# 3dhumangan/3DHumanGAN

Hardware: NVIDIA H100
Metric: images_per_sec_G_fwd_512x512 (higher is better)
Workload: dtype f32 (bf16x3 split on wgmma, fp32 accumulate)

## Files before the change

### 3dhumangan_b200/csrc/synth.cu

```cuda
#include "common.cuh"
#include "wgmma.cuh"

namespace hg {

constexpr int kC = 256;
constexpr int kSynThreads = 384;
constexpr int kSynStages = 2;
constexpr int kASlots = 2;
constexpr int kXSlots = 5;
constexpr int kXs = 3;
constexpr int kSs = 2;
constexpr uint32_t kAChunk = 128 * 128;
constexpr uint32_t kBStage = 256 * 128;
constexpr uint32_t kXSlice = 32 * 128 * 4;

struct SpadeArgs {
  const float* x;
  long x_bstride;
  const float* mod;
  const float* scsh;
  const float* p_lr;
  long p_stride;
  const float* p_bias;
  const uint8_t* wgb;
  const float* bgb;
  const uint8_t* wimg;
  const float* bias;
  const float* skip;
  long skip_bstride;
  float* out;
  double* stats;
  const float* rgb_w;
  const float* rgb_b;
  const float* rgb_in;
  float* rgb_out;
  int B, HW, Hg, Wg, Rh, Rw;
  int nkc;
  int xC;
  const float* x2;
  float slope;
  int cout;
  int out_pm;
  int act;
  const float* ascale;
  const float* rk_v;
  int rk_n;
  const float* mod2;
};

struct SynSmem {
  uint8_t* a_hi;
  uint8_t* a_lo;
  uint8_t* b_st;
  float* x_st;
  int xs_n, ss_n;
  float* tab_g1;
  float* tab_g0;
  float* tab_bias;
  float* tab_rgbw;
  float* tab_bgb;
  float* tab_as;
  float* st_sum;
  float* st_sq;
  uint64_t* bars;
};

template <bool kPixel>
__device__ __forceinline__ SynSmem carve(uint8_t* raw) {
  constexpr int kA = kPixel ? 3 : kASlots, kX = kPixel ? 3 : kXSlots;
  uint8_t* s = reinterpret_cast<uint8_t*>((reinterpret_cast<uintptr_t>(raw) + 1023) & ~uintptr_t(1023));
  SynSmem m;
  m.a_hi = s;
  m.a_lo = s + kA * kAChunk;
  m.b_st = s + 2 * kA * kAChunk;
  m.x_st = reinterpret_cast<float*>(m.b_st + kSynStages * kBStage);
  m.xs_n = kPixel ? 2 : kXs;
  m.ss_n = kPixel ? 1 : kSs;
  float* f = m.x_st + kX * (kXSlice / 4);
  m.tab_g1 = f; f += kC;
  m.tab_g0 = f; f += kC;
  m.tab_bias = f; f += kC;
  m.tab_rgbw = f; f += 3 * kC;
  m.tab_bgb = f; f += 512;
  m.tab_as = f; f += kC;
  m.st_sum = f; f += kC;
  m.st_sq = f; f += kC;
  m.bars = reinterpret_cast<uint64_t*>(f);
  return m;
}
constexpr uint32_t kSynSmemBytes = 2 * kASlots * kAChunk + kSynStages * kBStage + kXSlots * kXSlice +
                                   (kC * 9 + 512) * 4 + 24 * 8 + 1024;
constexpr uint32_t kPixSmemBytes = 2 * 3 * kAChunk + kSynStages * kBStage + 3 * kXSlice + (kC * 9 + 512) * 4 + 24 * 8 + 1024;
static_assert(kSynSmemBytes <= 232448 && kPixSmemBytes <= 232448, "shared memory budget");

enum { B_FULL = 0 , B_EMPTY = 2 , X_FULL = 4 , X_EMPTY = 12  };

__device__ __forceinline__ void rows_barrier() { named_barrier(1, 256); }

__device__ __forceinline__ float lrelu02(float v) { return v > 0.f ? v : 0.2f * v; }

__device__ __forceinline__ float reduce_2pi(float t) {
  const float y = t * 0.15915494309189535f;
  const float k = (y + 12582912.f) - 12582912.f;
  float r = fmaf(-k, 6.2831854820251465f, t);
  return fmaf(-k, -1.7484555314695172e-07f, r);
}
__device__ __forceinline__ float sin_red(float t) { return __sinf(reduce_2pi(t)); }
__device__ __forceinline__ float cos_red(float t) { return __cosf(reduce_2pi(t)); }
__device__ __forceinline__ float2 reduce_2pi2(float2 t) {
  const float2 y = fmul2(t, make_float2(0.15915494309189535f, 0.15915494309189535f));
  const float2 k = fadd2(fadd2(y, make_float2(12582912.f, 12582912.f)), make_float2(-12582912.f, -12582912.f));
  const float2 r = ffma2(k, make_float2(-6.2831854820251465f, -6.2831854820251465f), t);
  return ffma2(k, make_float2(1.7484555314695172e-07f, 1.7484555314695172e-07f), r);
}
__device__ __forceinline__ float2 sin_red2(float2 t) { const float2 r = reduce_2pi2(t); return make_float2(__sinf(r.x), __sinf(r.y)); }
__device__ __forceinline__ float2 cos_red2(float2 t) { const float2 r = reduce_2pi2(t); return make_float2(__cosf(r.x), __cosf(r.y)); }

struct TileMap {
  int T, first, stride, count;
  __device__ __forceinline__ void get(int it, int& b, int& ti) const {
    const int tile = first + it * stride;
    b = tile / T;
    ti = tile - b * T;
  }
};

__device__ __forceinline__ void init_common(const SpadeArgs& a, const SynSmem& m) {
  for (int i = threadIdx.x; i < kC; i += blockDim.x) {
    m.tab_bias[i] = a.bias[i];
    m.st_sum[i] = 0.f;
    m.st_sq[i] = 0.f;
  }
  if (a.rgb_w)
    for (int i = threadIdx.x; i < 3 * kC; i += blockDim.x) m.tab_rgbw[i] = a.rgb_w[i];
  if (threadIdx.x == 0) {
    for (int i = 0; i < kSynStages; ++i) {
      mbar_init(m.bars + B_FULL + i, 1);
      mbar_init(m.bars + B_EMPTY + i, 2);
    }
    for (int i = 0; i < m.xs_n + m.ss_n; ++i) {
      mbar_init(m.bars + X_FULL + i, 1);
      mbar_init(m.bars + X_EMPTY + i, 8);
    }
    fence_mbar_init();
  }
  __syncthreads();
}

template <int kPasses>
__device__ __forceinline__ void weight_producer_loop(const SynSmem& m, const uint8_t* img, int nstages, int num_my_tiles) {
  uint32_t st = 0, ph = 0;
  for (int t = 0; t < num_my_tiles; ++t)
    for (int s = 0; s < nstages; ++s) {
      if (kPasses == 1 && (s & 1)) continue;
      mbar_wait_backoff(m.bars + B_EMPTY + st, ph ^ 1);
      mbar_arrive_expect_tx(m.bars + B_FULL + st, kBStage);
      bulk_g2s(m.b_st + st * kBStage, img + static_cast<size_t>(s) * kBStage, kBStage, m.bars + B_FULL + st);
      if (++st == kSynStages) { st = 0; ph ^= 1; }
    }
}

struct Pipe {
  uint32_t st = 0, ph = 0, prev = ~0u;
};
template <int N, int kPasses>
__device__ __forceinline__ void pipe_chunk(const SynSmem& m, Pipe& p, float (&d)[N / 2], uint32_t a_hi, uint32_t a_lo, bool accumulate,
                                           int t) {
#pragma unroll
  for (int part = 0; part < (kPasses == 3 ? 2 : 1); ++part) {
    mbar_wait(m.bars + B_FULL + p.st, p.ph);
    acc_fence(d);
    wgmma_fence();
    const uint32_t bt = smem_u32(m.b_st + p.st * kBStage);
    if (part == 0) {
      wg_k64<N>(d, a_hi, bt, accumulate);
      if (kPasses == 3) wg_k64<N>(d, a_lo, bt, true);
    } else {
      wg_k64<N>(d, a_hi, bt, true);
    }
    wgmma_commit();
    wgmma_wait<1>();
    acc_fence(d);
    if (p.prev != ~0u && t == 0) mbar_arrive(m.bars + B_EMPTY + p.prev);
    p.prev = p.st;
    if (++p.st == kSynStages) { p.st = 0; p.ph ^= 1; }
  }
}
template <int N>
__device__ __forceinline__ void pipe_drain(const SynSmem& m, Pipe& p, float (&d)[N / 2], int t) {
  wgmma_wait<0>();
  acc_fence(d);
  if (p.prev != ~0u && t == 0) mbar_arrive(m.bars + B_EMPTY + p.prev);
  p.prev = ~0u;
}

__device__ __forceinline__ void ring_emit(const SynSmem& m, uint32_t& g, int base, int slots, const float* src) {
  const uint32_t slot = base + g % slots;
  mbar_wait_backoff(m.bars + X_EMPTY + slot, ((g / slots) & 1) ^ 1);
  mbar_arrive_expect_tx(m.bars + X_FULL + slot, kXSlice);
  bulk_g2s(m.x_st + slot * (kXSlice / 4), src, kXSlice, m.bars + X_FULL + slot);
  ++g;
}
__device__ __forceinline__ void x_producer_loop(const SpadeArgs& a, const SynSmem& m, const TileMap& tm) {
  uint32_t g = 0;
  for (int it = 0; it < tm.count; ++it) {
    int b, ti;
    tm.get(it, b, ti);
    const int per_src = a.xC / 32;
    const float* base = a.x + static_cast<long>(b) * a.x_bstride + static_cast<long>(ti) * a.xC * 128;
    const float* base2 = a.x2 ? a.x2 + (static_cast<long>(b) * tm.T + ti) * a.xC * 128 : nullptr;
    for (int j = 0; j < 2 * a.nkc; ++j)
      ring_emit(m, g, 0, m.xs_n, (j < per_src ? base : base2 - per_src * 32 * 128) + j * 32 * 128);
  }
}
__device__ __forceinline__ void skip_producer_loop(const SpadeArgs& a, const SynSmem& m, const TileMap& tm) {
  if (!a.skip) return;
  uint32_t g = 0;
  for (int it = 0; it < tm.count; ++it) {
    int b, ti;
    tm.get(it, b, ti);
    const float* base = a.skip + static_cast<long>(b) * a.skip_bstride + static_cast<long>(ti) * a.cout * 128;
    for (int j = 0; j < a.cout / 32; ++j) ring_emit(m, g, m.xs_n, m.ss_n, base + j * 32 * 128);
  }
}

__device__ __forceinline__ uint32_t ring_take(const SynSmem& m, uint32_t g, int base, int slots) {
  const uint32_t slot = base + g % slots;
  mbar_wait_sleep(m.bars + X_FULL + slot, (g / slots) & 1);
  return slot;
}
__device__ __forceinline__ void ring_release(const SynSmem& m, uint32_t slot) {
  __syncwarp();
  if ((threadIdx.x & 31) == 0) mbar_arrive(m.bars + X_EMPTY + slot);
}

__device__ __forceinline__ void take_x_pair(const SynSmem& m, uint32_t& xg, int h, int row, float (&dst)[32]) {
#pragma unroll
  for (int hh = 0; hh < 2; ++hh, ++xg) {
    const uint32_t xslot = ring_take(m, xg, 0, m.xs_n);
    if (hh == h) {
      const uint32_t xs = smem_u32(m.x_st + xslot * (kXSlice / 4)) + row * 4;
#pragma unroll
      for (int j = 0; j < 32; ++j) dst[j] = lds_f32(xs + j * 512);
    }
    ring_release(m, xslot);
  }
}

__device__ __forceinline__ void column_sums(float* st, int c0, const float (&v)[4][2]) {
  const int lane = threadIdx.x & 31, r = lane >> 2;
  const bool b2 = r & 4, b1 = r & 2, b0 = r & 1;
  float w[4], u[2];
#pragma unroll
  for (int i = 0; i < 4; ++i) {
    const float lo = v[i >> 1][i & 1], hi = v[(i + 4) >> 1][i & 1];
    w[i] = (b2 ? hi : lo) + __shfl_xor_sync(0xffffffffu, b2 ? lo : hi, 16);
  }
#pragma unroll
  for (int i = 0; i < 2; ++i)
    u[i] = (b1 ? w[i + 2] : w[i]) + __shfl_xor_sync(0xffffffffu, b1 ? w[i] : w[i + 2], 8);
  const float x = (b0 ? u[1] : u[0]) + __shfl_xor_sync(0xffffffffu, b0 ? u[0] : u[1], 4);
  atomicAdd(st + c0 + 8 * (r >> 1) + 2 * (lane & 3) + (r & 1), x);
}

template <bool kSkip>
__device__ __forceinline__ void epilogue_fwd(const SpadeArgs& a, const SynSmem& m, const float (&d)[128], int b, int ti, int T,
                                             int g, int t, uint32_t& sg) {
  const int HW = a.HW, cout = a.cout;
  const bool kRgb = a.rgb_w != nullptr, kStats = a.stats != nullptr;
  int row[2];
  bool valid[2];
#pragma unroll
  for (int i = 0; i < 2; ++i) {
    row[i] = g * 64 + frag_row(t, i);
    valid[i] = ti * 128 + row[i] < HW;
  }
  float* const otile = a.out + (static_cast<long>(b) * T + ti) * cout * 128;
  float r[2][3] = {{0.f, 0.f, 0.f}, {0.f, 0.f, 0.f}};
#pragma unroll
  for (int cg = 0; cg < 8; ++cg) {
    if (cg * 32 >= cout) break;
    float sk[2][4][2];
    if (kSkip) {
      const uint32_t slot = ring_take(m, sg, m.xs_n, m.ss_n);
      const float* xs = m.x_st + slot * (kXSlice / 4);
#pragma unroll
      for (int i = 0; i < 2; ++i)
#pragma unroll
        for (int jj = 0; jj < 4; ++jj)
#pragma unroll
          for (int e = 0; e < 2; ++e) sk[i][jj][e] = xs[(frag_col(t, jj, e)) * 128 + row[i]];
      ring_release(m, slot);
      ++sg;
    }
    float s1[4][2], s2[4][2];
#pragma unroll
    for (int jj = 0; jj < 4; ++jj)
#pragma unroll
      for (int e = 0; e < 2; ++e) {
        const int j = cg * 4 + jj, c = frag_col(t, j, e);
        const float bc = m.tab_bias[c];
        s1[jj][e] = 0.f;
        s2[jj][e] = 0.f;
#pragma unroll
        for (int i = 0; i < 2; ++i) {
          float v = d[4 * j + 2 * i + e] + bc;
          if (kSkip) v += sk[i][jj][e];
          if (valid[i]) otile[c * 128 + row[i]] = v;
          else v = 0.f;
          if (kRgb) {
#pragma unroll
            for (int k = 0; k < 3; ++k) r[i][k] = fmaf(v, m.tab_rgbw[k * kC + c], r[i][k]);
          }
          s1[jj][e] += v;
          s2[jj][e] = fmaf(v, v, s2[jj][e]);
        }
      }
    if (kStats) {
      column_sums(m.st_sum, cg * 32, s1);
      column_sums(m.st_sq, cg * 32, s2);
    }
  }
  if (kRgb) {
#pragma unroll
    for (int i = 0; i < 2; ++i) {
#pragma unroll
      for (int k = 0; k < 3; ++k) {
        r[i][k] += __shfl_xor_sync(0xffffffffu, r[i][k], 1);
        r[i][k] += __shfl_xor_sync(0xffffffffu, r[i][k], 2);
      }
      if ((t & 3) == 0 && valid[i]) {
        const int pix = ti * 128 + row[i];
#pragma unroll
        for (int k = 0; k < 3; ++k) {
          const long idx = (static_cast<long>(b) * 3 + k) * HW + pix;
          float o = r[i][k] + a.rgb_b[k];
          if (a.rgb_in) o += a.rgb_in[idx];
          a.rgb_out[idx] = o;
        }
      }
    }
  }
}

__device__ __forceinline__ void epilogue_fwd_any(const SpadeArgs& a, const SynSmem& m, const float (&d)[128], int b, int ti, int T,
                                                 int g, int t, uint32_t& sg) {
  if (a.skip) epilogue_fwd<true>(a, m, d, b, ti, T, g, t, sg);
  else epilogue_fwd<false>(a, m, d, b, ti, T, g, t, sg);
}

__device__ __forceinline__ void flush_fwd_stats(const SpadeArgs& a, const SynSmem& m) {
  rows_barrier();
  if (a.stats)
    for (int c = threadIdx.x; c < kC; c += 256) {
      atomicAdd(a.stats + c, static_cast<double>(m.st_sum[c]));
      atomicAdd(a.stats + kC + c, static_cast<double>(m.st_sq[c]));
    }
}

template <bool kSine, bool kRk, bool kPm>
__device__ __forceinline__ void epilogue_bwd(const SpadeArgs& a, const SynSmem& m, const float (&d)[128], int b, int ti, int T, int g,
                                             int t, uint32_t& sg) {
  const int HW = a.HW, cout = a.cout, rk_n = a.rk_n;
  const float mslope = a.slope;
  int row[2];
  bool valid[2];
  float rv[2][3] = {{0.f, 0.f, 0.f}, {0.f, 0.f, 0.f}};
#pragma unroll
  for (int i = 0; i < 2; ++i) {
    row[i] = g * 64 + frag_row(t, i);
    valid[i] = ti * 128 + row[i] < HW;
    if (kRk && valid[i]) {
      const float* rp = a.rk_v + static_cast<long>(b) * rk_n * HW + ti * 128 + row[i];
      rv[i][0] = rp[0];
      if (rk_n > 1) rv[i][1] = rp[HW];
      if (rk_n > 2) rv[i][2] = rp[2 * static_cast<long>(HW)];
    }
  }
  float* const otile = a.out + (static_cast<long>(b) * T + ti) * cout * 128;
#pragma unroll
  for (int cg = 0; cg < 8; ++cg) {
    if (cg * 32 >= cout) break;
    float xv[2][4][2];
    {
      const uint32_t slot = ring_take(m, sg, m.xs_n, m.ss_n);
      const float* xs = m.x_st + slot * (kXSlice / 4);
#pragma unroll
      for (int i = 0; i < 2; ++i)
#pragma unroll
        for (int jj = 0; jj < 4; ++jj)
#pragma unroll
          for (int e = 0; e < 2; ++e)
            xv[i][jj][e] = valid[i] ? xs[frag_col(t, jj, e) * 128 + row[i]] : 0.f;
      ring_release(m, slot);
      ++sg;
    }
    float s1[4][2], s2[4][2];
#pragma unroll
    for (int jj = 0; jj < 4; ++jj)
#pragma unroll
      for (int e = 0; e < 2; ++e) {
        const int j = cg * 4 + jj, c = frag_col(t, j, e);
        const float t1 = m.tab_g1[c], t0 = m.tab_g0[c];
        s1[jj][e] = 0.f;
        s2[jj][e] = 0.f;
#pragma unroll
        for (int i = 0; i < 2; ++i) {
          const float x = xv[i][jj][e];
          const float pre = fmaf(x, t1, t0);
          float acc = d[4 * j + 2 * i + e];
          if (kRk)
            acc = fmaf(rv[i][2], m.tab_rgbw[2 * kC + c], fmaf(rv[i][1], m.tab_rgbw[kC + c], fmaf(rv[i][0], m.tab_rgbw[c], acc)));
          const float mask = kSine ? cos_red(pre) : (pre > 0.f ? 1.f : mslope);
          const float dd = acc * mask;
          if (valid[i]) {
            if (kPm) a.out[(static_cast<long>(b) * HW + ti * 128 + row[i]) * cout + c] = dd;
            else otile[c * 128 + row[i]] = dd;
          }
          s1[jj][e] += dd;
          s2[jj][e] = fmaf(dd, x, s2[jj][e]);
        }
      }
    column_sums(m.st_sum, cg * 32, s1);
    column_sums(m.st_sq, cg * 32, s2);
  }
}

__device__ __forceinline__ void epilogue_bwd_any(const SpadeArgs& a, const SynSmem& m, const float (&d)[128], int b, int ti, int T,
                                                 int g, int t, uint32_t& sg) {
  if (a.act == 1) {
    if (a.rk_v) epilogue_bwd<true, true, false>(a, m, d, b, ti, T, g, t, sg);
    else epilogue_bwd<true, false, false>(a, m, d, b, ti, T, g, t, sg);
  } else {
    if (a.out_pm) epilogue_bwd<false, false, true>(a, m, d, b, ti, T, g, t, sg);
    else epilogue_bwd<false, false, false>(a, m, d, b, ti, T, g, t, sg);
  }
}

__device__ __forceinline__ void flush_bwd_sums(const SpadeArgs& a, const SynSmem& m, int b) {
  for (int c = threadIdx.x; c < a.cout; c += 256) {
    atomicAdd(a.stats + (static_cast<long>(b) * 2 + 0) * a.cout + c, static_cast<double>(m.st_sum[c]));
    atomicAdd(a.stats + (static_cast<long>(b) * 2 + 1) * a.cout + c, static_cast<double>(m.st_sq[c]));
    m.st_sum[c] = 0.f;
    m.st_sq[c] = 0.f;
  }
}

template <int kPasses, bool kBwd>
__global__ void __launch_bounds__(kSynThreads, 1) spade_const_kernel(SpadeArgs a) {
  extern __shared__ uint8_t smem_raw[];
  const SynSmem m = carve<false>(smem_raw);
  const int warp = threadIdx.x >> 5, lane = threadIdx.x & 31;
  init_common(a, m);
  TileMap tm;
  tm.T = (a.HW + 127) / 128;
  tm.first = blockIdx.x;
  tm.stride = gridDim.x;
  tm.count = (a.B * tm.T - static_cast<int>(blockIdx.x) + static_cast<int>(gridDim.x) - 1) / static_cast<int>(gridDim.x);

  if (warp < 8) {
    regs_inc<kMmaRegs>();
    const int g = warp >> 2, t = threadIdx.x & 127;
    const int q = 2 * g + (warp & 1), h = (warp >> 1) & 1;
    const int row = q * 32 + lane;
    int cur_b = -1;
    uint32_t acnt = 0;
    uint32_t xg = 0, sg = 0;
    Pipe p;
    float d[128];
    for (int it = 0; it < tm.count; ++it) {
      int b, ti;
      tm.get(it, b, ti);
      if (b != cur_b) {
        rows_barrier();
        if (kBwd && cur_b >= 0) flush_bwd_sums(a, m, cur_b);
        for (int i = threadIdx.x; i < kC; i += 256) {
          if (kBwd) {
            if (a.ascale) {
              const long ld = a.x2 ? 2 * kC : kC;
              m.tab_as[i] = a.ascale[static_cast<long>(b) * ld + i];
              if (a.x2) m.tab_bgb[i] = a.ascale[static_cast<long>(b) * ld + kC + i];
            }
            if (i < a.cout) {
              m.tab_g1[i] = a.mod ? a.mod[(static_cast<long>(b) * 2 + 0) * a.cout + i] : 1.f;
              m.tab_g0[i] = a.mod ? a.mod[(static_cast<long>(b) * 2 + 1) * a.cout + i] : 0.f;
            }
          } else {
            m.tab_g1[i] = a.mod ? a.mod[(static_cast<long>(b) * 2 + 0) * kC + i] : 1.f;
            m.tab_g0[i] = a.mod ? a.mod[(static_cast<long>(b) * 2 + 1) * kC + i] : 0.f;
            if (a.mod2) {
              m.tab_bgb[i] = a.mod2[(static_cast<long>(b) * 2 + 0) * kC + i];
              m.tab_bgb[kC + i] = a.mod2[(static_cast<long>(b) * 2 + 1) * kC + i];
            }
          }
        }
        rows_barrier();
        cur_b = b;
      }
      const bool valid = ti * 128 + row < a.HW;
      uint32_t tg1a = smem_u32(kBwd ? m.tab_as : m.tab_g1), tg0a = smem_u32(m.tab_g0);
      uint32_t tg1b = smem_u32(m.tab_bgb), tg0b = smem_u32(m.tab_bgb + kC);
      opaque(tg1a);
      opaque(tg0a);
      opaque(tg1b);
      opaque(tg0b);
      const float slope = a.slope;
      const bool sine = a.act == 1, scaled = kBwd && a.ascale != nullptr;
      const bool two_tables = kBwd ? (scaled && a.x2 != nullptr) : a.mod2 != nullptr;
#pragma unroll 1
      for (int kc = 0; kc < a.nkc; ++kc, ++acnt) {
        const int c0 = (kc * 64 + h * 32) & (kC - 1);
        const bool second = two_tables && kc * 64 >= kC;
        const uint32_t tg1 = second ? tg1b : tg1a, tg0 = second ? tg0b : tg0a;
        float cur[32];
        take_x_pair(m, xg, h, row, cur);
        const uint32_t slot = acnt & 1;
#pragma unroll
        for (int gi = 0; gi < 4; ++gi) {
          float y[8], t1[8], t0[8];
          if (!kBwd || scaled) lds8(tg1 + (c0 + gi * 8) * 4, t1);
          if (!kBwd) lds8(tg0 + (c0 + gi * 8) * 4, t0);
          if (kBwd) {
#pragma unroll
            for (int j = 0; j < 8; ++j) y[j] = scaled ? cur[gi * 8 + j] * t1[j] : cur[gi * 8 + j];
          } else if (sine) {
#pragma unroll
            for (int j = 0; j < 8; j += 2) {
              const float2 sv = sin_red2(ffma2(make_float2(cur[gi * 8 + j], cur[gi * 8 + j + 1]), make_float2(t1[j], t1[j + 1]),
                                               make_float2(t0[j], t0[j + 1])));
              y[j] = sv.x;
              y[j + 1] = sv.y;
            }
          } else {
            affine_lrelu8(cur + gi * 8, t1, t0, slope, y);
          }
          if (!valid) {
#pragma unroll
            for (int j = 0; j < 8; ++j) y[j] = 0.f;
          }
          store_a8<kPasses == 3>(m.a_hi + slot * kAChunk, m.a_lo + slot * kAChunk, row, h * 32 + gi * 8, y);
        }
        fence_proxy_async_smem();
        named_barrier(2 + g, 128);
        pipe_chunk<256, kPasses>(m, p, d, smem_u32(m.a_hi + slot * kAChunk) + g * 64 * 128,
                                 smem_u32(m.a_lo + slot * kAChunk) + g * 64 * 128, kc > 0, t);
      }
      pipe_drain<256>(m, p, d, t);
      if (kBwd) epilogue_bwd_any(a, m, d, b, ti, tm.T, g, t, sg);
      else epilogue_fwd_any(a, m, d, b, ti, tm.T, g, t, sg);
    }
    if (kBwd) {
      rows_barrier();
      if (cur_b >= 0) flush_bwd_sums(a, m, cur_b);
    } else {
      flush_fwd_stats(a, m);
    }
  } else {
    regs_dec<kProducerRegs>();
    if (lane == 0) {
      if (warp == 8) weight_producer_loop<kPasses>(m, a.wimg, 2 * a.nkc, tm.count);
      else if (warp == 9) x_producer_loop(a, m, tm);
      else if (warp == 10) skip_producer_loop(a, m, tm);
    }
  }
}

__device__ __forceinline__ void bilin(int dst, int in_size, float scale, int& i0, int& i1, float& l0, float& l1) {
  float src = scale * (static_cast<float>(dst) + 0.5f) - 0.5f;
  src = src < 0.f ? 0.f : src;
  i0 = static_cast<int>(src);
  i1 = i0 + (i0 < in_size - 1 ? 1 : 0);
  l1 = src - static_cast<float>(i0);
  l0 = 1.f - l1;
}

template <int kPasses>
__device__ __forceinline__ void pixel_weight_producer_loop(const SpadeArgs& a, const SynSmem& m, int num_my_tiles) {
  uint32_t st = 0, ph = 0;
  auto emit = [&](const uint8_t* src, uint32_t bytes) {
    mbar_wait_backoff(m.bars + B_EMPTY + st, ph ^ 1);
    mbar_arrive_expect_tx(m.bars + B_FULL + st, bytes);
    bulk_g2s(m.b_st + st * kBStage, src, bytes, m.bars + B_FULL + st);
    if (++st == kSynStages) { st = 0; ph ^= 1; }
  };
  for (int t = 0; t < num_my_tiles; ++t)
    for (int kc = 0; kc < 4; ++kc) {
      for (int k = 0; k < 2; ++k)
        for (int part = 0; part < (kPasses == 3 ? 2 : 1); ++part)
          emit(a.wgb + static_cast<size_t>(((kc >> 1) * 2 + k) * 2 + part) * kBStage + (kc & 1) * (kBStage / 2), kBStage / 2);
      for (int part = 0; part < (kPasses == 3 ? 2 : 1); ++part) emit(a.wimg + static_cast<size_t>(kc * 2 + part) * kBStage, kBStage);
    }
}

template <int kPasses>
__global__ void __launch_bounds__(kSynThreads, 1) spade_pixel_kernel(SpadeArgs a) {
  extern __shared__ uint8_t smem_raw[];
  const SynSmem m = carve<true>(smem_raw);
  const int warp = threadIdx.x >> 5, lane = threadIdx.x & 31;
  for (int i = threadIdx.x; i < kC; i += blockDim.x) {
    m.tab_g1[i] = a.scsh[i];
    m.tab_g0[i] = a.scsh[kC + i];
  }
  for (int i = threadIdx.x; i < 512; i += blockDim.x) m.tab_bgb[i] = a.bgb[i];
  init_common(a, m);
  TileMap tm;
  tm.T = (a.HW + 127) / 128;
  tm.first = blockIdx.x;
  tm.stride = gridDim.x;
  tm.count = (a.B * tm.T - static_cast<int>(blockIdx.x) + static_cast<int>(gridDim.x) - 1) / static_cast<int>(gridDim.x);
  const float sy = static_cast<float>(a.Rh) / static_cast<float>(a.Hg);
  const float sx = static_cast<float>(a.Rw) / static_cast<float>(a.Wg);

  if (warp < 8) {
    regs_inc<kMmaRegs>();
    const int g = warp >> 2, t = threadIdx.x & 127;
    const int q = 2 * g + (warp & 1), h = (warp >> 1) & 1;
    const int row = q * 32 + lane;
    uint8_t* const y_hi = m.a_hi + 2 * kAChunk;
    uint8_t* const y_lo = m.a_lo + 2 * kAChunk;
    uint32_t xg = 0, sg = 0;
    Pipe p;
    float d[128], e[64];
    for (int it = 0; it < tm.count; ++it) {
      int b, ti;
      tm.get(it, b, ti);
      const int pix = ti * 128 + row;
      const bool valid = pix < a.HW;
      {
        const int py = valid ? pix / a.Wg : 0, px = valid ? pix % a.Wg : 0;
        int y0, y1, x0, x1;
        float ly0, ly1, lx0, lx1;
        bilin(py, a.Rh, sy, y0, y1, ly0, ly1);
        bilin(px, a.Rw, sx, x0, x1, lx0, lx1);
        const float* base = a.p_lr + static_cast<long>(b) * a.Rh * a.Rw * a.p_stride;
        const float4* n00 = reinterpret_cast<const float4*>(base + (static_cast<long>(y0) * a.Rw + x0) * a.p_stride);
        const float4* n01 = reinterpret_cast<const float4*>(base + (static_cast<long>(y0) * a.Rw + x1) * a.p_stride);
        const float4* n10 = reinterpret_cast<const float4*>(base + (static_cast<long>(y1) * a.Rw + x0) * a.p_stride);
        const float4* n11 = reinterpret_cast<const float4*>(base + (static_cast<long>(y1) * a.Rw + x1) * a.p_stride);
        const float4* pb = a.p_bias ? reinterpret_cast<const float4*>(a.p_bias + static_cast<long>(b) * 128) : nullptr;
        const float2 lx0p = make_float2(lx0, lx0), lx1p = make_float2(lx1, lx1), ly0p = make_float2(ly0, ly0), ly1p = make_float2(ly1, ly1);
#pragma unroll 2
        for (int gi = 0; gi < 8; ++gi) {
          float y[8];
#pragma unroll
          for (int u = 0; u < 2; ++u) {
            const int f4 = h * 16 + gi * 2 + u;
            const float4 v00 = __ldg(n00 + f4), v01 = __ldg(n01 + f4), v10 = __ldg(n10 + f4), v11 = __ldg(n11 + f4);
            auto lerp2 = [&](float2 a, float2 b, float2 c, float2 d) {
              const float2 top = ffma2(b, lx1p, fmul2(a, lx0p));
              const float2 bot = ffma2(d, lx1p, fmul2(c, lx0p));
              return ffma2(top, ly0p, fmul2(bot, ly1p));
            };
            float2 lo2 = lerp2(make_float2(v00.x, v00.y), make_float2(v01.x, v01.y), make_float2(v10.x, v10.y), make_float2(v11.x, v11.y));
            float2 hi2 = lerp2(make_float2(v00.z, v00.w), make_float2(v01.z, v01.w), make_float2(v10.z, v10.w), make_float2(v11.z, v11.w));
            if (pb) {
              const float4 c4 = __ldg(pb + f4);
              lo2 = fadd2(lo2, make_float2(c4.x, c4.y));
              hi2 = fadd2(hi2, make_float2(c4.z, c4.w));
            }
            y[u * 4 + 0] = lo2.x; y[u * 4 + 1] = lo2.y; y[u * 4 + 2] = hi2.x; y[u * 4 + 3] = hi2.y;
          }
#pragma unroll
          for (int j = 0; j < 8; ++j) y[j] = valid ? fmaxf(y[j], 0.f) : 0.f;
          store_a8<kPasses == 3>(m.a_hi + h * kAChunk, m.a_lo + h * kAChunk, row, gi * 8, y);
        }
        fence_proxy_async_smem();
        named_barrier(2 + g, 128);
      }
      int frow[2];
      bool fvalid[2];
#pragma unroll
      for (int i = 0; i < 2; ++i) {
        frow[i] = g * 64 + frag_row(t, i);
        fvalid[i] = ti * 128 + frow[i] < a.HW;
      }
#pragma unroll 1
      for (int kc = 0; kc < 4; ++kc) {
        for (int k = 0; k < 2; ++k)
          pipe_chunk<128, kPasses>(m, p, e, smem_u32(m.a_hi + k * kAChunk) + g * 64 * 128, smem_u32(m.a_lo + k * kAChunk) + g * 64 * 128,
                                   k > 0, t);
        pipe_drain<128>(m, p, e, t);
        const uint32_t s0 = ring_take(m, xg, 0, m.xs_n), s1 = ring_take(m, xg + 1, 0, m.xs_n);
        xg += 2;
        const float* xs0 = m.x_st + s0 * (kXSlice / 4);
        const float* xs1 = m.x_st + s1 * (kXSlice / 4);
        const int col = (kc >> 1) * 256 + (kc & 1) * 128;
#pragma unroll
        for (int j = 0; j < 8; ++j) {
          const int c = frag_col(t, j, 0), ch = kc * 64 + c;
          const float* xs = j < 4 ? xs0 : xs1;
#pragma unroll
          for (int i = 0; i < 2; ++i) {
            float y2[2];
#pragma unroll
            for (int u = 0; u < 2; ++u) {
              const float gam = e[4 * j + 2 * i + u] + m.tab_bgb[col + c + u];
              const float bet = e[4 * (j + 8) + 2 * i + u] + m.tab_bgb[col + 64 + c + u];
              const float xn = fmaf(xs[((c + u) & 31) * 128 + frow[i]], m.tab_g1[ch + u], m.tab_g0[ch + u]);
              const float v = fmaf(xn, gam, bet);
              y2[u] = fvalid[i] ? fmaxf(v, 0.2f * v) : 0.f;
            }
            uint32_t hb, lb;
            split_bf16x2(y2[0], y2[1], hb, lb);
            const uint32_t off = sw128_offset(frow[i], c);
            asm volatile("st.shared.b32 [%0], %1;" ::"r"(smem_u32(y_hi) + off), "r"(hb));
            if (kPasses == 3) asm volatile("st.shared.b32 [%0], %1;" ::"r"(smem_u32(y_lo) + off), "r"(lb));
          }
        }
        ring_release(m, s0);
        ring_release(m, s1);
        fence_proxy_async_smem();
        named_barrier(2 + g, 128);
        pipe_chunk<256, kPasses>(m, p, d, smem_u32(y_hi) + g * 64 * 128, smem_u32(y_lo) + g * 64 * 128, kc > 0, t);
      }
      pipe_drain<256>(m, p, d, t);
      epilogue_fwd_any(a, m, d, b, ti, tm.T, g, t, sg);
    }
    flush_fwd_stats(a, m);
  } else {
    regs_dec<kProducerRegs>();
    if (lane == 0) {
      if (warp == 8) pixel_weight_producer_loop<kPasses>(a, m, tm.count);
      else if (warp == 9) x_producer_loop(a, m, tm);
      else if (warp == 10) skip_producer_loop(a, m, tm);
    }
  }
}

__global__ void bn_finalize_kernel(const double* __restrict__ stats, double count_in, const double* __restrict__ count_ptr,
                                   const float* __restrict__ weight,
                                   const float* __restrict__ bias, float* running_mean, float* running_var,
                                   int training, float eps, float momentum, const float* __restrict__ gb, int B,
                                   float* __restrict__ scsh, float* __restrict__ mod) {
  const int c = threadIdx.x;
  float mean, var;
  const double count = count_ptr ? count_ptr[0] : count_in;
  if (training) {
    const double mu = stats[c] / count;
    double v = stats[kC + c] / count - mu * mu;
    v = v < 0 ? 0 : v;
    mean = static_cast<float>(mu);
    var = static_cast<float>(v);
    if (running_mean) {
      const double unb = count > 1 ? v * count / (count - 1) : v;
      running_mean[c] = (1.f - momentum) * running_mean[c] + momentum * mean;
      running_var[c] = (1.f - momentum) * running_var[c] + momentum * static_cast<float>(unb);
    }
  } else {
    mean = running_mean[c];
    var = running_var[c];
  }
  const float sc = weight[c] * rsqrtf(var + eps);
  const float sh = bias[c] - mean * sc;
  if (scsh) {
    scsh[c] = sc;
    scsh[kC + c] = sh;
  }
  if (mod && gb) {
    for (int b = 0; b < B; ++b) {
      const float G = gb[(static_cast<long>(b) * 2 + 0) * kC + c];
      const float Bt = gb[(static_cast<long>(b) * 2 + 1) * kC + c];
      mod[(static_cast<long>(b) * 2 + 0) * kC + c] = sc * G;
      mod[(static_cast<long>(b) * 2 + 1) * kC + c] = fmaf(sh, G, Bt);
    }
  }
}

__global__ void synth_input_kernel(const float* __restrict__ w, const float* __restrict__ bias,
                                   const float* __restrict__ ic, const float* __restrict__ jc, int Hg, int Wg,
                                   float* __restrict__ x0, double* __restrict__ stats, double batch_mult) {
  const int c = blockIdx.y;
  const int HW = Hg * Wg;
  const float w0 = w[c * 2 + 0], w1 = w[c * 2 + 1], bb = bias[c];
  float s1 = 0.f, s2 = 0.f;
  for (int p = blockIdx.x * blockDim.x + threadIdx.x; p < HW; p += gridDim.x * blockDim.x) {
    const float v = sinf(fmaf(w1, jc[p % Wg], fmaf(w0, ic[p / Wg], bb)));
    x0[(static_cast<long>(p >> 7) * kC + c) * 128 + (p & 127)] = v;
    s1 += v;
    s2 += v * v;
  }
  __shared__ float r1[8], r2[8];
  for (int o = 16; o > 0; o >>= 1) {
    s1 += __shfl_xor_sync(0xffffffffu, s1, o);
    s2 += __shfl_xor_sync(0xffffffffu, s2, o);
  }
  if ((threadIdx.x & 31) == 0) { r1[threadIdx.x >> 5] = s1; r2[threadIdx.x >> 5] = s2; }
  __syncthreads();
  if (threadIdx.x == 0 && stats) {
    float t1 = 0.f, t2 = 0.f;
    for (int i = 0; i < static_cast<int>(blockDim.x >> 5); ++i) { t1 += r1[i]; t2 += r2[i]; }
    atomicAdd(stats + c, static_cast<double>(t1) * batch_mult);
    atomicAdd(stats + kC + c, static_cast<double>(t2) * batch_mult);
  }
}

}

extern "C" {

int hg_spade_conv(const float* x, long x_bstride, const float* mod, const float* scsh, const float* p_lr,
                  long p_stride, const float* p_bias, const void* wgb, const float* bgb, const void* wimg, const float* bias, const float* skip,
                  float* out, double* stats, const float* rgb_w, const float* rgb_b, const float* rgb_in,
                  float* rgb_out, int B, int C, int Hg, int Wg, int Rh, int Rw, int passes, void* stream) {
  HG_REQUIRE(C == hg::kC, "hg_spade_conv: only %d channels are supported (got %d)", hg::kC, C);
  HG_REQUIRE(x && wimg && bias && out, "hg_spade_conv: null pointer");
  HG_REQUIRE((mod != nullptr) != (p_lr != nullptr), "hg_spade_conv: give exactly one of mod (const style) / p_lr (pixel style)");
  HG_REQUIRE(passes == 1 || passes == 3, "hg_spade_conv: passes must be 1 or 3");
  HG_REQUIRE(B > 0 && Hg > 0 && Wg > 0, "hg_spade_conv: bad shape");
  HG_REQUIRE(!rgb_w || (rgb_b && rgb_out), "hg_spade_conv: rgb_b / rgb_out missing");
  if (p_lr) {
    HG_REQUIRE(scsh && wgb && bgb && Rh > 0 && Rw > 0, "hg_spade_conv: pixel-style arguments missing");
    HG_REQUIRE((reinterpret_cast<uintptr_t>(p_lr) & 15) == 0 && p_stride >= 128 && (p_stride & 3) == 0,
               "hg_spade_conv: p_lr must be 16-byte aligned with a row stride >= 128 that is a multiple of 4");
    HG_REQUIRE(!p_bias || (reinterpret_cast<uintptr_t>(p_bias) & 15) == 0, "hg_spade_conv: p_bias must be 16-byte aligned");
  }
  hg::SpadeArgs a{x, x_bstride, mod, scsh, p_lr, p_stride, p_bias, static_cast<const uint8_t*>(wgb), bgb,
                  static_cast<const uint8_t*>(wimg), bias, skip,
                  static_cast<long>((Hg * Wg + 127) / 128) * hg::kC * 128, out, stats, rgb_w, rgb_b, rgb_in, rgb_out,
                  B, Hg * Wg, Hg, Wg, Rh, Rw};
  a.nkc = 4; a.xC = hg::kC; a.x2 = nullptr; a.slope = 0.2f; a.cout = hg::kC; a.out_pm = 0;
  const int tiles = B * ((Hg * Wg + 127) / 128);
  const int grid = tiles < hg::num_sms() ? tiles : hg::num_sms();
  auto st = static_cast<cudaStream_t>(stream);
#define HG_LAUNCH(KERNEL, SMEM)                                                                                   \
  do {                                                                                                            \
    cudaError_t e = cudaFuncSetAttribute(KERNEL, cudaFuncAttributeMaxDynamicSharedMemorySize, SMEM);               \
    if (e != cudaSuccess) { hg::set_error("hg_spade_conv: smem opt-in failed: %s", cudaGetErrorString(e)); return 2; } \
    KERNEL<<<grid, hg::kSynThreads, SMEM, st>>>(a);                                                               \
  } while (0)
  if (mod) {
    if (passes == 3) HG_LAUNCH((hg::spade_const_kernel<3, false>), hg::kSynSmemBytes); else HG_LAUNCH((hg::spade_const_kernel<1, false>), hg::kSynSmemBytes);
  } else {
    if (passes == 3) HG_LAUNCH(hg::spade_pixel_kernel<3>, hg::kPixSmemBytes); else HG_LAUNCH(hg::spade_pixel_kernel<1>, hg::kPixSmemBytes);
  }
#undef HG_LAUNCH
  return hg::check_launch("hg_spade_conv");
}

static int launch_blocked_gemm(const hg::SpadeArgs& a, int passes, bool bwd, cudaStream_t st, const char* who) {
  const int tiles = a.B * ((a.HW + 127) / 128);
  const int grid = tiles < hg::num_sms() ? tiles : hg::num_sms();
  cudaError_t e;
#define HG_LAUNCH_G(KERNEL)                                                                             \
  do {                                                                                                  \
    e = cudaFuncSetAttribute(KERNEL, cudaFuncAttributeMaxDynamicSharedMemorySize, hg::kSynSmemBytes);   \
    if (e == cudaSuccess) KERNEL<<<grid, hg::kSynThreads, hg::kSynSmemBytes, st>>>(a);                   \
  } while (0)
  if (bwd) {
    if (passes == 3) HG_LAUNCH_G((hg::spade_const_kernel<3, true>)); else HG_LAUNCH_G((hg::spade_const_kernel<1, true>));
  } else {
    if (passes == 3) HG_LAUNCH_G((hg::spade_const_kernel<3, false>)); else HG_LAUNCH_G((hg::spade_const_kernel<1, false>));
  }
#undef HG_LAUNCH_G
  if (e != cudaSuccess) { hg::set_error("%s: smem opt-in failed: %s", who, cudaGetErrorString(e)); return 2; }
  return hg::check_launch(who);
}

int hg_spade_bwd_dgrad(const float* dout, const float* x, long x_bstride, const float* mod, const void* wimg_t, float* dpre,
                       double* sums, int B, int C, int Hg, int Wg, int passes, void* stream) {
  HG_REQUIRE(C == hg::kC, "hg_spade_bwd_dgrad: only %d channels are supported (got %d)", hg::kC, C);
  HG_REQUIRE(dout && x && mod && wimg_t && dpre && sums, "hg_spade_bwd_dgrad: null pointer");
  HG_REQUIRE(passes == 1 || passes == 3, "hg_spade_bwd_dgrad: passes must be 1 or 3");
  HG_REQUIRE(B > 0 && Hg > 0 && Wg > 0, "hg_spade_bwd_dgrad: bad shape");
  const long T = (Hg * Wg + 127) / 128;
  hg::SpadeArgs a{};
  a.x = dout;
  a.x_bstride = T * hg::kC * 128;
  a.mod = mod;
  a.wimg = static_cast<const uint8_t*>(wimg_t);
  a.bias = mod;
  a.skip = x;
  a.skip_bstride = x_bstride;
  a.out = dpre;
  a.stats = sums;
  a.B = B; a.HW = Hg * Wg; a.Hg = Hg; a.Wg = Wg;
  a.nkc = 4; a.xC = hg::kC; a.slope = 0.2f; a.cout = hg::kC;
  return launch_blocked_gemm(a, passes, true, static_cast<cudaStream_t>(stream), "hg_spade_bwd_dgrad");
}

int hg_conv1x1_blocked(const float* x, int Cin, const void* wimg, const float* bias, float* out, int B, int Hg, int Wg,
                       int passes, void* stream) {
  HG_REQUIRE(x && wimg && bias && out, "hg_conv1x1_blocked: null pointer");
  HG_REQUIRE(Cin == 64 || Cin == 128 || Cin == 256, "hg_conv1x1_blocked: Cin must be 64, 128 or 256 (got %d)", Cin);
  HG_REQUIRE(passes == 1 || passes == 3, "hg_conv1x1_blocked: passes must be 1 or 3");
  HG_REQUIRE(B > 0 && Hg > 0 && Wg > 0, "hg_conv1x1_blocked: bad shape");
  const long T = (Hg * Wg + 127) / 128;
  hg::SpadeArgs a{};
  a.x = x;
  a.x_bstride = T * Cin * 128;
  a.wimg = static_cast<const uint8_t*>(wimg);
  a.bias = bias;
  a.skip_bstride = T * hg::kC * 128;
  a.out = out;
  a.B = B; a.HW = Hg * Wg; a.Hg = Hg; a.Wg = Wg;
  a.nkc = Cin / 64; a.xC = Cin; a.slope = 1.f; a.cout = hg::kC;
  return launch_blocked_gemm(a, passes, false, static_cast<cudaStream_t>(stream), "hg_conv1x1_blocked");
}

int hg_act_conv1x1_blocked(const float* x, const float* x2, const float* mod, int act, const void* wimg, const float* bias,
                           float* out, int B, int Hg, int Wg, int passes, void* stream) {
  HG_REQUIRE(x && mod && wimg && bias && out, "hg_act_conv1x1_blocked: null pointer");
  HG_REQUIRE(act == 0 || act == 1, "hg_act_conv1x1_blocked: act must be 0 (LeakyReLU 0.2) or 1 (sine)");
  HG_REQUIRE(passes == 1 || passes == 3, "hg_act_conv1x1_blocked: passes must be 1 or 3");
  HG_REQUIRE(B > 0 && Hg > 0 && Wg > 0, "hg_act_conv1x1_blocked: bad shape");
  const long T = (Hg * Wg + 127) / 128;
  hg::SpadeArgs a{};
  a.x = x;
  a.x_bstride = T * hg::kC * 128;
  a.x2 = x2;
  a.mod = mod;
  a.wimg = static_cast<const uint8_t*>(wimg);
  a.bias = bias;
  a.skip_bstride = T * hg::kC * 128;
  a.out = out;
  a.B = B; a.HW = Hg * Wg; a.Hg = Hg; a.Wg = Wg;
  a.nkc = x2 ? 8 : 4; a.xC = hg::kC; a.slope = 0.2f; a.cout = hg::kC; a.act = act;
  return launch_blocked_gemm(a, passes, false, static_cast<cudaStream_t>(stream), "hg_act_conv1x1_blocked");
}

int hg_blocked_conv_wide(const float* x, const float* x2, const float* mod, const float* mod2, int act, float slope,
                         const void* wimg, const float* bias, const float* skip, float* out, double* stats,
                         const float* rgb_w, const float* rgb_b, const float* rgb_in, float* rgb_out, int B, int Hg, int Wg,
                         int passes, void* stream) {
  HG_REQUIRE(x && wimg && bias && out, "hg_blocked_conv_wide: null pointer");
  HG_REQUIRE(act == 0 || act == 1, "hg_blocked_conv_wide: act must be 0 (LeakyReLU(slope)) or 1 (sine)");
  HG_REQUIRE(!mod2 || (mod && x2), "hg_blocked_conv_wide: mod2 needs mod and a second source");
  HG_REQUIRE(!rgb_w || (rgb_b && rgb_out), "hg_blocked_conv_wide: rgb_b / rgb_out missing");
  HG_REQUIRE(passes == 1 || passes == 3, "hg_blocked_conv_wide: passes must be 1 or 3");
  HG_REQUIRE(B > 0 && Hg > 0 && Wg > 0, "hg_blocked_conv_wide: bad shape");
  const long T = (Hg * Wg + 127) / 128;
  hg::SpadeArgs a{};
  a.x = x;
  a.x_bstride = T * hg::kC * 128;
  a.x2 = x2;
  a.mod = mod;
  a.mod2 = mod2;
  a.wimg = static_cast<const uint8_t*>(wimg);
  a.bias = bias;
  a.skip = skip;
  a.skip_bstride = T * hg::kC * 128;
  a.out = out;
  a.stats = stats;
  a.rgb_w = rgb_w; a.rgb_b = rgb_b; a.rgb_in = rgb_in; a.rgb_out = rgb_out;
  a.B = B; a.HW = Hg * Wg; a.Hg = Hg; a.Wg = Wg;
  a.nkc = x2 ? 8 : 4; a.xC = hg::kC; a.slope = slope; a.cout = hg::kC; a.act = act;
  return launch_blocked_gemm(a, passes, false, static_cast<cudaStream_t>(stream), "hg_blocked_conv_wide");
}

int hg_conv1x1_blocked_bwd(const float* g, const float* g2, const float* aux, const float* mod, const void* wimg_t,
                           float* out, double* sums, int Cout, float slope, int pixel_major, int act, const float* ascale,
                           const float* rk_w, const float* rk_v, int rk_n, int B, int Hg, int Wg, int passes,
                           void* stream) {
  HG_REQUIRE(act == 0 || act == 1, "hg_conv1x1_blocked_bwd: act must be 0 (LeakyReLU/ReLU mask) or 1 (cosine)");
  HG_REQUIRE(!rk_v || (rk_w && rk_n >= 1 && rk_n <= 3 && Cout == 256), "hg_conv1x1_blocked_bwd: bad rank-k term");
  HG_REQUIRE(g && aux && wimg_t && out && sums, "hg_conv1x1_blocked_bwd: null pointer");
  HG_REQUIRE(Cout == 128 || Cout == 256, "hg_conv1x1_blocked_bwd: Cout must be 128 or 256 (got %d)", Cout);
  HG_REQUIRE(!pixel_major || Cout == 128, "hg_conv1x1_blocked_bwd: the pixel-major output is built for Cout == 128");
  HG_REQUIRE(!(act == 1 && pixel_major) && !(act == 0 && rk_v),
             "hg_conv1x1_blocked_bwd: compiled epilogues are sine [+ rank-k term] / LeakyReLU [+ pixel-major output]");
  HG_REQUIRE(passes == 1 || passes == 3, "hg_conv1x1_blocked_bwd: passes must be 1 or 3");
  HG_REQUIRE(B > 0 && Hg > 0 && Wg > 0, "hg_conv1x1_blocked_bwd: bad shape");
  const long T = (Hg * Wg + 127) / 128;
  hg::SpadeArgs a{};
  a.x = g;
  a.x_bstride = T * hg::kC * 128;
  a.x2 = g2;
  a.mod = mod;
  a.wimg = static_cast<const uint8_t*>(wimg_t);
  a.bias = static_cast<const float*>(wimg_t);
  a.skip = aux;
  a.skip_bstride = T * Cout * 128;
  a.out = out;
  a.stats = sums;
  a.B = B; a.HW = Hg * Wg; a.Hg = Hg; a.Wg = Wg;
  a.nkc = g2 ? 8 : 4; a.xC = hg::kC; a.slope = slope; a.cout = Cout; a.out_pm = pixel_major;
  a.act = act; a.ascale = ascale; a.rgb_w = rk_v ? rk_w : nullptr; a.rk_v = rk_v; a.rk_n = rk_n;
  return launch_blocked_gemm(a, passes, true, static_cast<cudaStream_t>(stream), "hg_conv1x1_blocked_bwd");
}

int hg_bn_finalize(const double* stats, double count, const double* count_dev, const float* weight, const float* bias, float* running_mean,
                   float* running_var, int training, float eps, float momentum, const float* gb, int B, int C,
                   float* scsh, float* mod, void* stream) {
  HG_REQUIRE(C == hg::kC, "hg_bn_finalize: only %d channels are supported (got %d)", hg::kC, C);
  HG_REQUIRE(weight && bias && (scsh || mod), "hg_bn_finalize: null pointer");
  HG_REQUIRE(training ? (stats != nullptr && (count > 0 || count_dev)) : (running_mean && running_var),
             "hg_bn_finalize: statistics missing");
  hg::bn_finalize_kernel<<<1, hg::kC, 0, static_cast<cudaStream_t>(stream)>>>(
      stats, count, count_dev, weight, bias, running_mean, running_var, training, eps, momentum, gb, B, scsh, mod);
  return hg::check_launch("hg_bn_finalize");
}

int hg_synth_input(const float* w, const float* bias, const float* ic, const float* jc, int C, int Hg, int Wg,
                   float* x0, double* stats, int batch, void* stream) {
  HG_REQUIRE(C == hg::kC, "hg_synth_input: only %d channels are supported (got %d)", hg::kC, C);
  HG_REQUIRE(w && bias && ic && jc && x0, "hg_synth_input: null pointer");
  const int HW = Hg * Wg;
  int bx = (HW + 255) / 256;
  if (bx > 32) bx = 32;
  dim3 grid(bx, C);
  hg::synth_input_kernel<<<grid, 256, 0, static_cast<cudaStream_t>(stream)>>>(w, bias, ic, jc, Hg, Wg, x0, stats,
                                                                              static_cast<double>(batch));
  return hg::check_launch("hg_synth_input");
}

}
```

Baseline: 100.1.

## Split weight stages into half-width slots with deeper four-slot ring

The weight ring now uses four 16KB slots instead of two 32KB stages. Each N=256 MMA chunk is issued as two N=128 halves, and each half waits on its own slot. This should let weight TMA loads run further ahead and release buffers sooner at the same smem footprint, but it adds more barrier waits and more wgmma commits. The change also adds globaltimer phase stamping, which is compiled out by default.

```diff
diff --git a/3dhumangan_b200/csrc/synth.cu b/3dhumangan_b200/csrc/synth.cu
--- a/3dhumangan_b200/csrc/synth.cu
+++ b/3dhumangan_b200/csrc/synth.cu
@@ -5,13 +5,14 @@
 
 constexpr int kC = 256;
 constexpr int kSynThreads = 384;
-constexpr int kSynStages = 2;
+constexpr int kWSlots = 4;
 constexpr int kASlots = 2;
 constexpr int kXSlots = 5;
 constexpr int kXs = 3;
 constexpr int kSs = 2;
 constexpr uint32_t kAChunk = 128 * 128;
 constexpr uint32_t kBStage = 256 * 128;
+constexpr uint32_t kWSlot = 128 * 128;
 constexpr uint32_t kXSlice = 32 * 128 * 4;
 
 struct SpadeArgs {
@@ -73,7 +74,7 @@
   m.a_hi = s;
   m.a_lo = s + kA * kAChunk;
   m.b_st = s + 2 * kA * kAChunk;
-  m.x_st = reinterpret_cast<float*>(m.b_st + kSynStages * kBStage);
+  m.x_st = reinterpret_cast<float*>(m.b_st + kWSlots * kWSlot);
   m.xs_n = kPixel ? 2 : kXs;
   m.ss_n = kPixel ? 1 : kSs;
   float* f = m.x_st + kX * (kXSlice / 4);
@@ -88,12 +89,12 @@
   m.bars = reinterpret_cast<uint64_t*>(f);
   return m;
 }
-constexpr uint32_t kSynSmemBytes = 2 * kASlots * kAChunk + kSynStages * kBStage + kXSlots * kXSlice +
+constexpr uint32_t kSynSmemBytes = 2 * kASlots * kAChunk + kWSlots * kWSlot + kXSlots * kXSlice +
                                    (kC * 9 + 512) * 4 + 24 * 8 + 1024;
-constexpr uint32_t kPixSmemBytes = 2 * 3 * kAChunk + kSynStages * kBStage + 3 * kXSlice + (kC * 9 + 512) * 4 + 24 * 8 + 1024;
+constexpr uint32_t kPixSmemBytes = 2 * 3 * kAChunk + kWSlots * kWSlot + 3 * kXSlice + (kC * 9 + 512) * 4 + 24 * 8 + 1024;
 static_assert(kSynSmemBytes <= 232448 && kPixSmemBytes <= 232448, "shared memory budget");
 
-enum { B_FULL = 0 , B_EMPTY = 2 , X_FULL = 4 , X_EMPTY = 12  };
+enum { B_FULL = 0 , B_EMPTY = 4 , X_FULL = 8 , X_EMPTY = 13  };
 
 __device__ __forceinline__ void rows_barrier() { named_barrier(1, 256); }
 
@@ -125,6 +126,31 @@
   }
 };
 
+enum { PH_TILE = 0, PH_WAIT_X, PH_BUILD, PH_WAIT_W, PH_MMA, PH_WAIT_S, PH_EPI, PH_TABLE };
+#ifdef HG_SPADE_STAMPS
+constexpr int kStampCtas = 4, kStampEvents = 16384;
+__device__ unsigned long long g_spade_stamps[kStampCtas][kStampEvents];
+struct Clk {
+  unsigned long long* buf = nullptr;
+  uint32_t n = 0;
+  __device__ __forceinline__ void start() {
+    if (threadIdx.x == 0 && blockIdx.x < kStampCtas) buf = g_spade_stamps[blockIdx.x];
+  }
+  __device__ __forceinline__ void mark(int phase) {
+    if (buf && n < kStampEvents) {
+      unsigned long long v;
+      asm volatile("mov.u64 %0, %%globaltimer;" : "=l"(v));
+      buf[n++] = (v & ~0xFull) | static_cast<unsigned long long>(phase);
+    }
+  }
+};
+#else
+struct Clk {
+  __device__ __forceinline__ void start() {}
+  __device__ __forceinline__ void mark(int) {}
+};
+#endif
+
 __device__ __forceinline__ void init_common(const SpadeArgs& a, const SynSmem& m) {
   for (int i = threadIdx.x; i < kC; i += blockDim.x) {
     m.tab_bias[i] = a.bias[i];
@@ -134,7 +160,7 @@
   if (a.rgb_w)
     for (int i = threadIdx.x; i < 3 * kC; i += blockDim.x) m.tab_rgbw[i] = a.rgb_w[i];
   if (threadIdx.x == 0) {
-    for (int i = 0; i < kSynStages; ++i) {
+    for (int i = 0; i < kWSlots; ++i) {
       mbar_init(m.bars + B_FULL + i, 1);
       mbar_init(m.bars + B_EMPTY + i, 2);
     }
@@ -147,49 +173,65 @@
   __syncthreads();
 }
 
+struct WeightFill {
+  uint32_t st = 0, ph = 0;
+  __device__ __forceinline__ void emit(const SynSmem& m, const uint8_t* src) {
+    mbar_wait_backoff(m.bars + B_EMPTY + st, ph ^ 1);
+    mbar_arrive_expect_tx(m.bars + B_FULL + st, kWSlot);
+    bulk_g2s(m.b_st + st * kWSlot, src, kWSlot, m.bars + B_FULL + st);
+    if (++st == kWSlots) { st = 0; ph ^= 1; }
+  }
+};
 template <int kPasses>
 __device__ __forceinline__ void weight_producer_loop(const SynSmem& m, const uint8_t* img, int nstages, int num_my_tiles) {
-  uint32_t st = 0, ph = 0;
+  WeightFill f;
   for (int t = 0; t < num_my_tiles; ++t)
     for (int s = 0; s < nstages; ++s) {
       if (kPasses == 1 && (s & 1)) continue;
-      mbar_wait_backoff(m.bars + B_EMPTY + st, ph ^ 1);
-      mbar_arrive_expect_tx(m.bars + B_FULL + st, kBStage);
-      bulk_g2s(m.b_st + st * kBStage, img + static_cast<size_t>(s) * kBStage, kBStage, m.bars + B_FULL + st);
-      if (++st == kSynStages) { st = 0; ph ^= 1; }
+      for (int h = 0; h < 2; ++h) f.emit(m, img + static_cast<size_t>(s) * kBStage + h * kWSlot);
     }
 }
 
 struct Pipe {
   uint32_t st = 0, ph = 0, prev = ~0u;
 };
+template <int kPasses>
+__device__ __forceinline__ void pipe_slot(const SynSmem& m, Pipe& p, float (&d)[64], uint32_t a_hi, uint32_t a_lo, bool hi_part,
+                                          bool accumulate, int t, Clk& clk) {
+  mbar_wait(m.bars + B_FULL + p.st, p.ph);
+  clk.mark(PH_WAIT_W);
+  acc_fence(d);
+  wgmma_fence();
+  const uint32_t bt = smem_u32(m.b_st + p.st * kWSlot);
+  if (hi_part) {
+    wg_k64<128>(d, a_hi, bt, accumulate);
+    if (kPasses == 3) wg_k64<128>(d, a_lo, bt, true);
+  } else {
+    wg_k64<128>(d, a_hi, bt, true);
+  }
+  wgmma_commit();
+  wgmma_wait<1>();
+  acc_fence(d);
+  clk.mark(PH_MMA);
+  if (p.prev != ~0u && t == 0) mbar_arrive(m.bars + B_EMPTY + p.prev);
+  p.prev = p.st;
+  if (++p.st == kWSlots) { p.st = 0; p.ph ^= 1; }
+}
 template <int N, int kPasses>
 __device__ __forceinline__ void pipe_chunk(const SynSmem& m, Pipe& p, float (&d)[N / 2], uint32_t a_hi, uint32_t a_lo, bool accumulate,
-                                           int t) {
-#pragma unroll
-  for (int part = 0; part < (kPasses == 3 ? 2 : 1); ++part) {
-    mbar_wait(m.bars + B_FULL + p.st, p.ph);
-    acc_fence(d);
-    wgmma_fence();
-    const uint32_t bt = smem_u32(m.b_st + p.st * kBStage);
-    if (part == 0) {
-      wg_k64<N>(d, a_hi, bt, accumulate);
-      if (kPasses == 3) wg_k64<N>(d, a_lo, bt, true);
-    } else {
-      wg_k64<N>(d, a_hi, bt, true);
-    }
-    wgmma_commit();
-    wgmma_wait<1>();
-    acc_fence(d);
-    if (p.prev != ~0u && t == 0) mbar_arrive(m.bars + B_EMPTY + p.prev);
-    p.prev = p.st;
-    if (++p.st == kSynStages) { p.st = 0; p.ph ^= 1; }
-  }
+                                           int t, Clk& clk) {
+#pragma unroll
+  for (int part = 0; part < (kPasses == 3 ? 2 : 1); ++part)
+#pragma unroll
+    for (int h = 0; h < N / 128; ++h)
+      pipe_slot<kPasses>(m, p, *reinterpret_cast<float(*)[64]>(d + 64 * h), a_hi, a_lo, part == 0, part == 0 ? accumulate : true, t,
+                         clk);
 }
 template <int N>
-__device__ __forceinline__ void pipe_drain(const SynSmem& m, Pipe& p, float (&d)[N / 2], int t) {
+__device__ __forceinline__ void pipe_drain(const SynSmem& m, Pipe& p, float (&d)[N / 2], int t, Clk& clk) {
   wgmma_wait<0>();
   acc_fence(d);
+  clk.mark(PH_MMA);
   if (p.prev != ~0u && t == 0) mbar_arrive(m.bars + B_EMPTY + p.prev);
   p.prev = ~0u;
 }
@@ -234,14 +276,16 @@
   if ((threadIdx.x & 31) == 0) mbar_arrive(m.bars + X_EMPTY + slot);
 }
 
-__device__ __forceinline__ void take_x_pair(const SynSmem& m, uint32_t& xg, int h, int row, float (&dst)[32]) {
+__device__ __forceinline__ void take_x_pair(const SynSmem& m, uint32_t& xg, int h, int row, float (&dst)[32], Clk& clk) {
 #pragma unroll
   for (int hh = 0; hh < 2; ++hh, ++xg) {
     const uint32_t xslot = ring_take(m, xg, 0, m.xs_n);
+    clk.mark(PH_WAIT_X);
     if (hh == h) {
       const uint32_t xs = smem_u32(m.x_st + xslot * (kXSlice / 4)) + row * 4;
 #pragma unroll
       for (int j = 0; j < 32; ++j) dst[j] = lds_f32(xs + j * 512);
+      clk.mark(PH_BUILD);
     }
     ring_release(m, xslot);
   }
@@ -265,7 +309,7 @@
 
 template <bool kSkip>
 __device__ __forceinline__ void epilogue_fwd(const SpadeArgs& a, const SynSmem& m, const float (&d)[128], int b, int ti, int T,
-                                             int g, int t, uint32_t& sg) {
+                                             int g, int t, uint32_t& sg, Clk& clk) {
   const int HW = a.HW, cout = a.cout;
   const bool kRgb = a.rgb_w != nullptr, kStats = a.stats != nullptr;
   int row[2];
@@ -282,7 +326,9 @@
     if (cg * 32 >= cout) break;
     float sk[2][4][2];
     if (kSkip) {
+      clk.mark(PH_EPI);
       const uint32_t slot = ring_take(m, sg, m.xs_n, m.ss_n);
+      clk.mark(PH_WAIT_S);
       const float* xs = m.x_st + slot * (kXSlice / 4);
 #pragma unroll
       for (int i = 0; i < 2; ++i)
@@ -341,12 +387,13 @@
       }
     }
   }
+  clk.mark(PH_EPI);
 }
 
 __device__ __forceinline__ void epilogue_fwd_any(const SpadeArgs& a, const SynSmem& m, const float (&d)[128], int b, int ti, int T,
-                                                 int g, int t, uint32_t& sg) {
-  if (a.skip) epilogue_fwd<true>(a, m, d, b, ti, T, g, t, sg);
-  else epilogue_fwd<false>(a, m, d, b, ti, T, g, t, sg);
+                                                 int g, int t, uint32_t& sg, Clk& clk) {
+  if (a.skip) epilogue_fwd<true>(a, m, d, b, ti, T, g, t, sg, clk);
+  else epilogue_fwd<false>(a, m, d, b, ti, T, g, t, sg, clk);
 }
 
 __device__ __forceinline__ void flush_fwd_stats(const SpadeArgs& a, const SynSmem& m) {
@@ -467,10 +514,13 @@
     uint32_t acnt = 0;
     uint32_t xg = 0, sg = 0;
     Pipe p;
+    Clk clk;
+    if (!kBwd) clk.start();
     float d[128];
     for (int it = 0; it < tm.count; ++it) {
       int b, ti;
       tm.get(it, b, ti);
+      clk.mark(PH_TILE);
       if (b != cur_b) {
         rows_barrier();
         if (kBwd && cur_b >= 0) flush_bwd_sums(a, m, cur_b);
@@ -496,6 +546,7 @@
         }
         rows_barrier();
         cur_b = b;
+        clk.mark(PH_TABLE);
       }
       const bool valid = ti * 128 + row < a.HW;
       uint32_t tg1a = smem_u32(kBwd ? m.tab_as : m.tab_g1), tg0a = smem_u32(m.tab_g0);
@@ -513,7 +564,7 @@
         const bool second = two_tables && kc * 64 >= kC;
         const uint32_t tg1 = second ? tg1b : tg1a, tg0 = second ? tg0b : tg0a;
         float cur[32];
-        take_x_pair(m, xg, h, row, cur);
+        take_x_pair(m, xg, h, row, cur, clk);
         const uint32_t slot = acnt & 1;
 #pragma unroll
         for (int gi = 0; gi < 4; ++gi) {
@@ -542,12 +593,13 @@
         }
         fence_proxy_async_smem();
         named_barrier(2 + g, 128);
+        clk.mark(PH_BUILD);
         pipe_chunk<256, kPasses>(m, p, d, smem_u32(m.a_hi + slot * kAChunk) + g * 64 * 128,
-                                 smem_u32(m.a_lo + slot * kAChunk) + g * 64 * 128, kc > 0, t);
+                                 smem_u32(m.a_lo + slot * kAChunk) + g * 64 * 128, kc > 0, t, clk);
       }
-      pipe_drain<256>(m, p, d, t);
+      pipe_drain<256>(m, p, d, t, clk);
       if (kBwd) epilogue_bwd_any(a, m, d, b, ti, tm.T, g, t, sg);
-      else epilogue_fwd_any(a, m, d, b, ti, tm.T, g, t, sg);
+      else epilogue_fwd_any(a, m, d, b, ti, tm.T, g, t, sg, clk);
     }
     if (kBwd) {
       rows_barrier();
@@ -576,19 +628,14 @@
 
 template <int kPasses>
 __device__ __forceinline__ void pixel_weight_producer_loop(const SpadeArgs& a, const SynSmem& m, int num_my_tiles) {
-  uint32_t st = 0, ph = 0;
-  auto emit = [&](const uint8_t* src, uint32_t bytes) {
-    mbar_wait_backoff(m.bars + B_EMPTY + st, ph ^ 1);
-    mbar_arrive_expect_tx(m.bars + B_FULL + st, bytes);
-    bulk_g2s(m.b_st + st * kBStage, src, bytes, m.bars + B_FULL + st);
-    if (++st == kSynStages) { st = 0; ph ^= 1; }
-  };
+  WeightFill f;
   for (int t = 0; t < num_my_tiles; ++t)
     for (int kc = 0; kc < 4; ++kc) {
       for (int k = 0; k < 2; ++k)
         for (int part = 0; part < (kPasses == 3 ? 2 : 1); ++part)
-          emit(a.wgb + static_cast<size_t>(((kc >> 1) * 2 + k) * 2 + part) * kBStage + (kc & 1) * (kBStage / 2), kBStage / 2);
-      for (int part = 0; part < (kPasses == 3 ? 2 : 1); ++part) emit(a.wimg + static_cast<size_t>(kc * 2 + part) * kBStage, kBStage);
+          f.emit(m, a.wgb + static_cast<size_t>(((kc >> 1) * 2 + k) * 2 + part) * kBStage + (kc & 1) * kWSlot);
+      for (int part = 0; part < (kPasses == 3 ? 2 : 1); ++part)
+        for (int h = 0; h < 2; ++h) f.emit(m, a.wimg + static_cast<size_t>(kc * 2 + part) * kBStage + h * kWSlot);
     }
 }
 
@@ -620,10 +667,13 @@
     uint8_t* const y_lo = m.a_lo + 2 * kAChunk;
     uint32_t xg = 0, sg = 0;
     Pipe p;
+    Clk clk;
+    clk.start();
     float d[128], e[64];
     for (int it = 0; it < tm.count; ++it) {
       int b, ti;
       tm.get(it, b, ti);
+      clk.mark(PH_TILE);
       const int pix = ti * 128 + row;
       const bool valid = pix < a.HW;
       {
@@ -666,6 +716,7 @@
         }
         fence_proxy_async_smem();
         named_barrier(2 + g, 128);
+        clk.mark(PH_BUILD);
       }
       int frow[2];
       bool fvalid[2];
@@ -678,10 +729,11 @@
       for (int kc = 0; kc < 4; ++kc) {
         for (int k = 0; k < 2; ++k)
           pipe_chunk<128, kPasses>(m, p, e, smem_u32(m.a_hi + k * kAChunk) + g * 64 * 128, smem_u32(m.a_lo + k * kAChunk) + g * 64 * 128,
-                                   k > 0, t);
-        pipe_drain<128>(m, p, e, t);
+                                   k > 0, t, clk);
+        pipe_drain<128>(m, p, e, t, clk);
         const uint32_t s0 = ring_take(m, xg, 0, m.xs_n), s1 = ring_take(m, xg + 1, 0, m.xs_n);
         xg += 2;
+        clk.mark(PH_WAIT_X);
         const float* xs0 = m.x_st + s0 * (kXSlice / 4);
         const float* xs1 = m.x_st + s1 * (kXSlice / 4);
         const int col = (kc >> 1) * 256 + (kc & 1) * 128;
@@ -711,10 +763,11 @@
         ring_release(m, s1);
         fence_proxy_async_smem();
         named_barrier(2 + g, 128);
-        pipe_chunk<256, kPasses>(m, p, d, smem_u32(y_hi) + g * 64 * 128, smem_u32(y_lo) + g * 64 * 128, kc > 0, t);
+        clk.mark(PH_BUILD);
+        pipe_chunk<256, kPasses>(m, p, d, smem_u32(y_hi) + g * 64 * 128, smem_u32(y_lo) + g * 64 * 128, kc > 0, t, clk);
       }
-      pipe_drain<256>(m, p, d, t);
-      epilogue_fwd_any(a, m, d, b, ti, tm.T, g, t, sg);
+      pipe_drain<256>(m, p, d, t, clk);
+      epilogue_fwd_any(a, m, d, b, ti, tm.T, g, t, sg, clk);
     }
     flush_fwd_stats(a, m);
   } else {
@@ -1003,4 +1056,14 @@
   return hg::check_launch("hg_synth_input");
 }
 
-}
+#ifdef HG_SPADE_STAMPS
+int hg_spade_stamps_take(unsigned long long* dst) {
+  if (dst && cudaMemcpyFromSymbol(dst, hg::g_spade_stamps, sizeof(hg::g_spade_stamps)) != cudaSuccess) return -1;
+  void* p = nullptr;
+  if (cudaGetSymbolAddress(&p, hg::g_spade_stamps) != cudaSuccess || cudaMemset(p, 0, sizeof(hg::g_spade_stamps)) != cudaSuccess)
+    return -1;
+  return hg::kStampEvents;
+}
+#endif
+
+}
```

After: 103.7, median of 6. +3.6%, better.
